# brown-palm/goal-force

Measured on AMD Instinct MI355X. Metric: frames_per_sec (81-frame video / (50-step denoise loop + VAE decode), Wan2.2-I2V-A14B 832x480x81f), higher is better.
Workload: dtype bf16

## Files before the change

### goal_force_amd/csrc/gf_abi.hip

```cpp
#include "gf_common.h"
#include <cstdarg>
#include <cstdio>
#include <cstdlib>
#include <cstring>

static thread_local char g_err[512] = "";

void gf_set_error(const char* fmt, ...) {
    va_list ap;
    va_start(ap, fmt);
    vsnprintf(g_err, sizeof(g_err), fmt, ap);
    va_end(ap);
}

extern "C" GF_API const char* gf_version(void) { return "goalforce-hip 0.1.0 gfx950"; }
extern "C" GF_API const char* gf_last_error(void) { return g_err; }
extern "C" GF_API int gf_abi_version(void) { return GF_ABI_VERSION; }

static GfOptions g_options;

const GfOptions& gf_options() { return g_options; }

namespace {
struct OptionSlot {
    const char* name;
    std::atomic<int> GfOptions::*field;
    int lo, hi, dflt;
};
const OptionSlot kSlots[] = {
    {"prefer_8wave", &GfOptions::prefer_8wave, 0, 1, 0}, {"a4_stagger", &GfOptions::a4_stagger, 0, 1 << 20, 2},
    {"a4_group_m", &GfOptions::a4_group_m, 0, 64, 0},    {"conv_nb", &GfOptions::conv_nb, 0, 2, 0},
    {"conv_gather", &GfOptions::conv_gather, 0, 1, 0},   {"vae_rms3", &GfOptions::vae_rms3, 0, 1, 1},
    {"conv_direct", &GfOptions::conv_direct, 0, 1, 1},
};
}

extern "C" GF_API int gf_set_option(const char* name, int value) {
    GF_CHECK_ARG(name, "gf_set_option: null name");
    for (const OptionSlot& s : kSlots)
        if (strcmp(name, s.name) == 0) {
            (g_options.*(s.field)).store(value < s.lo ? s.lo : (value > s.hi ? s.hi : value), std::memory_order_relaxed);
            return GF_OK;
        }
    gf_set_error("gf_set_option: unknown option '%s'", name);
    return GF_ERR_INVALID_ARG;
}

extern "C" GF_API int gf_get_option(const char* name, int* value) {
    GF_CHECK_ARG(name && value, "gf_get_option: null argument");
    for (const OptionSlot& s : kSlots)
        if (strcmp(name, s.name) == 0) {
            *value = (g_options.*(s.field)).load(std::memory_order_relaxed);
            return GF_OK;
        }
    gf_set_error("gf_get_option: unknown option '%s'", name);
    return GF_ERR_INVALID_ARG;
}

extern "C" GF_API void gf_reset_options(void) {
    for (const OptionSlot& s : kSlots) (g_options.*(s.field)).store(s.dflt, std::memory_order_relaxed);
}
```

### goal_force_amd/csrc/gf_attention.hip

```cpp
#include "gf_mfma_frame.h"
#include <cstdlib>

namespace {

constexpr int QB = 256;
constexpr int KVB = 64;
constexpr int HD = 128;
constexpr int KV_TILE_BYTES = KVB * HD * 2;

constexpr int K3_RING = 2;
constexpr int K3_DMA0 = 10;
constexpr int K3_DMAS = 8;

struct AttnArgs {
    const u16* q;
    const u16* k;
    const u16* v;
    u16* o;
    int q_len, kv_len, heads, n_qblocks;
    long q_stride, k_stride, v_stride, o_stride;
    float scale_log2e;
    unsigned long long* dbg;
    float* lse;
    const u16* vt;
    long kv_pad;
    float last_key_bias;
    const int* row_ptr;
    const int* tile_idx;
    const int* head_map;
    int n_maps;
};

constexpr int AT2_THREADS = 512;
constexpr int AT2_V_BASE = 2 * KV_TILE_BYTES;
constexpr int AT2_LDS = 4 * KV_TILE_BYTES;

__device__ __forceinline__ void mfma32(f32x16& acc, const bf16x8& a, const bf16x8& b) {
    acc = __builtin_amdgcn_mfma_f32_32x32x16_bf16(a, b, acc, 0, 0, 0);
}

template <bool VT>
__global__ __launch_bounds__(AT2_THREADS, 2) void flash_attn_fwd_kernel2(const AttnArgs p) {
    extern __shared__ __attribute__((aligned(16))) char smem[];
    GF_LDS char* lds = (GF_LDS char*)smem;
    const int tid = threadIdx.x;
    const int lane = tid & 63;
    const int wave = __builtin_amdgcn_readfirstlane(tid >> 6);
    const int r = lane & 31, h = lane >> 5;
    int head, qb;
    {
        const int pid = blockIdx.x;
        if ((p.heads & 7) == 0) {
            const int xcd = pid & 7, idx = pid >> 3;
            head = xcd + 8 * (idx / p.n_qblocks);
            qb = idx % p.n_qblocks;
        } else {
            head = pid / p.n_qblocks;
            qb = pid % p.n_qblocks;
        }
    }
    const int q0 = qb * QB + wave * 32;

    bf16x8 qf[8];
// ... 379 lines not shown
        GF_LDS char* ob = lds + wave * 8192;
#pragma unroll
        for (int d = 0; d < 4; ++d)
#pragma unroll
            for (int rg = 0; rg < 4; ++rg) {
                u32x2 pk;
                pk[0] = pack2bf(oacc[d][4 * rg + 0] * inv, oacc[d][4 * rg + 1] * inv);
                pk[1] = pack2bf(oacc[d][4 * rg + 2] * inv, oacc[d][4 * rg + 3] * inv);
                *(GF_LDS u32x2*)(ob + r * 256 + (((4 * d + rg) ^ (r & 15)) << 4) + 8 * h) = pk;
            }
        asm volatile("s_waitcnt lgkmcnt(0)" ::: "memory");
#pragma unroll
        for (int it = 0; it < 8; ++it) {
            const int row = 4 * it + (lane >> 4), ch = lane & 15;
            const u16x8 v8 = *(GF_LDS u16x8*)(ob + row * 256 + ((ch ^ (row & 15)) << 4));
            if (q0 + row < p.q_len)
                *reinterpret_cast<u16x8*>(p.o + (long)(q0 + row) * p.o_stride + head * HD + 8 * ch) = v8;
        }
    }
}

constexpr int K3_NQ = 2;
template <int NQ> struct At3 {
    static constexpr int WAVES = 16 / NQ, THREADS = 64 * WAVES, ROWS = 16 * NQ, PIECES = NQ;
    static constexpr int SLOTS = 32 * NQ;
};
constexpr int AT3_V_BASE = 2 * KV_TILE_BYTES;
constexpr int AT3_LDS = 4 * KV_TILE_BYTES;

__device__ __forceinline__ void mfma16(f32x4& acc, const bf16x8& a, const bf16x8& b) {
    acc = __builtin_amdgcn_mfma_f32_16x16x32_bf16(a, b, acc, 0, 0, 0);
}

template <int NQ, bool SPARSE>
__global__ __launch_bounds__(At3<NQ>::THREADS, (NQ == 2 ? 2 : 1)) void flash_attn_fwd_kernel3(const AttnArgs p) {
    constexpr int NP = At3<NQ>::PIECES, NW = At3<NQ>::WAVES, RW = At3<NQ>::ROWS, NS = At3<NQ>::SLOTS;
    extern __shared__ __attribute__((aligned(16))) char smem[];
    GF_LDS char* lds = (GF_LDS char*)smem;
    const int tid = threadIdx.x;
    const int lane = tid & 63;
    const int wave = __builtin_amdgcn_readfirstlane(tid >> 6);
    const int r = lane & 15, g = lane >> 4;
    int head, qb0;
    gf_xcd_head_block(blockIdx.x, p.heads, p.n_qblocks, head, qb0);
    const int q0 = qb0 * QB + wave * RW;

    int vt_last = 0;
    bf16x8 qf[NQ][4];
#pragma unroll
    for (int qb = 0; qb < NQ; ++qb) {
        const int qr = min(q0 + 16 * qb + r, p.q_len - 1);
        const u16* qp = p.q + (long)qr * p.q_stride + head * HD + 8 * g;
#pragma unroll
        for (int ks = 0; ks < 4; ++ks) {
            qf[qb][ks] = *reinterpret_cast<const bf16x8*>(qp + 32 * ks);
        }
    }

    const int dma_r = lane >> 4;
    unsigned k_off0, vt_off0;
    {
        const int row = 4 * wave + dma_r;
        const int lch = (lane & 15) ^ (row & 15);
        k_off0 = ((unsigned)row * (unsigned)p.k_stride + head * HD + lch * 8) * 2u;
        const int vrow = 8 * wave + (lane >> 3);
        const int vch = (lane & 7) ^ ((vrow >> 1) & 7);
        vt_off0 = (unsigned)(((long)head * HD + vrow) * p.kv_pad + vch * 8) * 2u;
    }
    const unsigned kstep = KVB * (unsigned)p.k_stride * 2u;
    const unsigned k_piece = 4u * NW * (unsigned)p.k_stride * 2u, vt_piece = 8u * NW * (unsigned)p.kv_pad * 2u;
    typedef __attribute__((ext_vector_type(4))) unsigned u32x4s;
    auto make_srd = [](const void* base) {
        const unsigned long b = (unsigned long)base;
        u32x4s s;
        s[0] = (unsigned)b;
        s[1] = (unsigned)(b >> 32) & 0xffffu;
        s[2] = 0xffffffffu;
        s[3] = 0x00020000u;
// ... 96 lines not shown
    };

    auto qk_plain = [&](auto par_c) __attribute__((always_inline)) {
        constexpr int PAR = decltype(par_c)::value;
#pragma unroll
        for (int kb = 0; kb < 4; ++kb)
#pragma unroll
            for (int qb = 0; qb < NQ; ++qb) sc[PAR][kb][qb] = negm[qb];
#pragma unroll
        for (int ks = 0; ks < 4; ++ks)
#pragma unroll
            for (int kb = 0; kb < 4; ++kb) {
                const bf16x8 kf = *(GF_LDS bf16x8*)(lds + koff[ks] + kb * 4096 + PAR * KV_TILE_BYTES);
#pragma unroll
                for (int qb = 0; qb < NQ; ++qb) mfma_qk(sc[PAR][kb][qb], kf, qf[qb][ks]);
            }
    };
    auto pv_plain = [&](auto buf_c) __attribute__((always_inline)) {
        constexpr int BUF = decltype(buf_c)::value;
#pragma unroll
        for (int kk = 0; kk < 2; ++kk)
#pragma unroll
            for (int db = 0; db < 8; ++db) {
                const bf16x8 vf = *(GF_LDS bf16x8*)(lds + voff[kk] + db * 2048 + BUF * KV_TILE_BYTES);
#pragma unroll
                for (int qb = 0; qb < NQ; ++qb) mfma_pv(oacc[db][qb], vf, pf(kk, qb));
            }
#pragma unroll
        for (int kk = 0; kk < 2; ++kk)
#pragma unroll
            for (int qb = 0; qb < NQ; ++qb) mfma_pv(oacc[NDB - 1][qb], ones, pf(kk, qb));
    };
    auto apply_pending = [&]() __attribute__((always_inline)) {
        if (pend) {
    #pragma unroll
            for (int db = 0; db < NDB; ++db)
#pragma unroll
                for (int qb = 0; qb < NQ; ++qb)
#pragma unroll
                    for (int e = 0; e < 4; ++e) oacc[db][qb][e] *= alpha_pend[qb];
            pend = false;
        }
    };
    auto new_max = [&](auto par_c, const float (&mx)[NQ], bool first) {
        constexpr int PAR = decltype(par_c)::value;
        float over = mx[0];
#pragma unroll
        for (int qb = 1; qb < NQ; ++qb) over = fmaxf(over, mx[qb]);
        constexpr float QUIET = 6.0f;
        const bool quiet = __all(over <= QUIET);
        if (first || !quiet) {
#pragma unroll
            for (int qb = 0; qb < NQ; ++qb) {
                float d = mx[qb];
                d = fmaxf(d, __shfl_xor(d, 16));
                d = fmaxf(d, __shfl_xor(d, 32));
                if (!first) d = fmaxf(d, 0.f);
                const float m_new = d - negm[qb][0];
                const float alpha = __builtin_amdgcn_exp2f(-d);
#pragma unroll
                for (int kb = 0; kb < 4; ++kb)
#pragma unroll
                    for (int e = 0; e < 4; ++e) sc[PAR][kb][qb][e] -= d;
#pragma unroll
                for (int e = 0; e < 4; ++e) negm[qb][e] = -m_new;
                alpha_pend[qb] = alpha;
            }
            pend = !first;
        }
    };
    auto mask_ragged = [&](auto par_c, int t) __attribute__((always_inline)) {
        constexpr int PAR = decltype(par_c)::value;
        if (ragged && t == (SPARSE ? nt_all : nt) - 1) {
#pragma unroll
            for (int kb = 0; kb < 4; ++kb)
#pragma unroll
                for (int j = 0; j < 4; ++j)
                    if (t * KVB + 16 * kb + 4 * g + j >= p.kv_len) {
#pragma unroll
                        for (int qb = 0; qb < NQ; ++qb) sc[PAR][kb][qb][j] = -INFINITY;
                    }
        }
    };
    auto softmax_plain = [&](auto par_c, int t, int pos) __attribute__((always_inline)) {
        constexpr int PAR = decltype(par_c)::value;
        mask_ragged(par_c, t);
        float mx[NQ];
#pragma unroll
        for (int qb = 0; qb < NQ; ++qb) {
            mx[qb] = sc[PAR][0][qb][0];
#pragma unroll
            for (int kb = 0; kb < 4; ++kb)
#pragma unroll
                for (int j = 0; j < 4; ++j) mx[qb] = fmaxf(mx[qb], sc[PAR][kb][qb][j]);
        }
        new_max(par_c, mx, pos == 0);
#pragma unroll
        for (int qb = 0; qb < NQ; ++qb) {
#pragma unroll
            for (int kb = 0; kb < 4; ++kb)
#pragma unroll
                for (int j = 0; j < 4; j += 2) {
                    const float p0 = __builtin_amdgcn_exp2f(sc[PAR][kb][qb][j]);
                    const float p1 = __builtin_amdgcn_exp2f(sc[PAR][kb][qb][j + 1]);
                    pfw[kb >> 1][qb][(kb & 1) * 2 + (j >> 1)] = pack2bf(p0, p1);
                }
        }
    };

    constexpr int RING = K3_RING;
    bf16x8 fr[RING];
    auto frag_load = [&](auto f_c, auto par_c) __attribute__((always_inline)) {
        constexpr int F = decltype(f_c)::value, PAR = decltype(par_c)::value;
        if constexpr (F < 16) {
            constexpr int kk = F >> 3, db = F & 7;
            fr[F % RING] = *(GF_LDS bf16x8*)(lds + voff[kk] + db * 2048 + (1 - PAR) * KV_TILE_BYTES);
        } else if constexpr (F < 32) {
            constexpr int ks = (F - 16) >> 2, kb = (F - 16) & 3;
            fr[F % RING] = *(GF_LDS bf16x8*)(lds + koff[ks] + kb * 4096 + (1 - PAR) * KV_TILE_BYTES);
        }
    };
    auto mfma_op = [&](auto s_c, auto par_c) __attribute__((always_inline)) {
        constexpr int S = decltype(s_c)::value, PAR = decltype(par_c)::value;
        constexpr int F = S / NQ, qb = (F & 1) ? NQ - 1 - S % NQ : S % NQ;
        if constexpr (F < 16) {
            constexpr int kk = F >> 3, db = F & 7;
            mfma_pv(oacc[db][qb], fr[F % RING], pf(kk, qb));
        } else {
            constexpr int ks = (F - 16) >> 2, kb = (F - 16) & 3;
            if constexpr (ks == 0) {
                mfma_qk_first(sc[1 - PAR][kb][qb], fr[F % RING], qf[qb][ks], negm[qb]);
            } else {
                mfma_qk(sc[1 - PAR][kb][qb], fr[F % RING], qf[qb][ks]);
            }
        }
    };
    auto dma_slot = [&](auto s_c, auto par_c, int tv, int tk) __attribute__((always_inline)) {
        constexpr int S = decltype(s_c)::value, PAR = decltype(par_c)::value;
        if constexpr (S >= K3_DMA0 && (S - K3_DMA0) % K3_DMAS == 0 && (S - K3_DMA0) / K3_DMAS < 2 * NP) {
            constexpr int i = (S - K3_DMA0) / K3_DMAS;
            if constexpr (i < NP) {
                stage_piece(1, tv, PAR, i);
            } else {
                stage_piece(0, tk, PAR, i - NP);
            }
        }
    };
    auto phase = [&](auto par_c, int pidx) __attribute__((always_inline)) {
        constexpr int PAR = decltype(par_c)::value;
        apply_pending();
        gf_static_for<0, RING - 1>([&](auto f_c) { frag_load(f_c, par_c); });
        float mx[NQ];
#pragma unroll
        for (int qb = 0; qb < NQ; ++qb) mx[qb] = -INFINITY;
        gf_static_for<0, 4 * NQ>([&](auto s_c) {
            constexpr int S = decltype(s_c)::value;
            mfma_op(s_c, par_c);
            if constexpr (S % NQ == 0) frag_load(std::integral_constant<int, S / NQ + RING - 1>{}, par_c);
            {
                constexpr int kb = S / NQ, qb = S % NQ;
                const f32x4& v = sc[PAR][kb][qb];
                mx[qb] = fmaxf(fmaxf(mx[qb], v[0]), v[1]);
                mx[qb] = fmaxf(fmaxf(mx[qb], v[2]), v[3]);
            }
            __builtin_amdgcn_sched_barrier(0);
        });
        new_max(par_c, mx, false);
        float pe[2];
        gf_static_for<4 * NQ, NS>([&](auto s_c) {
            constexpr int S = decltype(s_c)::value;
            mfma_op(s_c, par_c);
            if constexpr (S == 8 * NQ - 1 || S == 16 * NQ - 1) {
#pragma unroll
                for (int qb = 0; qb < NQ; ++qb) mfma_pv(oacc[NDB - 1][qb], ones, pf(S / (8 * NQ), qb));
            }
            if constexpr (S % NQ == 0) frag_load(std::integral_constant<int, S / NQ + RING - 1>{}, par_c);
            dma_slot(s_c, par_c, SPARSE ? w0 : pidx, SPARSE ? w2 : pidx + 2);
            if constexpr (S >= 8 * NQ) {
                constexpr int T = (S - 8 * NQ) % 3, e = ((S - 8 * NQ) / 3) * 2 + (T == 2 ? 1 : T);
                constexpr int kk = e / (8 * NQ), qb = (e >> 3) % NQ, kb = 2 * kk + ((e >> 2) & 1), j = e & 3;
                if constexpr (T != 2) {
                    asm volatile("v_exp_f32 %0, %1" : "=v"(pe[T]) : "v"(sc[PAR][kb][qb][j]));
                } else {
                    unsigned w;
                    asm volatile("v_cvt_pk_bf16_f32 %0, %1, %2" : "=v"(w) : "v"(pe[0]), "v"(pe[1]));
                    pfw[kk][qb][(kb & 1) * 2 + (j >> 1)] = w;
                }
            }
            __builtin_amdgcn_sched_barrier(0);
        });
        if constexpr (SPARSE) {
            w0 = w1;
            w1 = w2;
            w2 = tile_clamp(w_next);
            w_next = tile_raw(pidx + 4);
        }
        asm volatile("s_waitcnt vmcnt(0)" ::: "memory");
        __syncthreads();
    };

// ... 15 lines not shown
    if (nt > 1) qk_plain(C1{});
    asm volatile("s_waitcnt vmcnt(0)" ::: "memory");
    __syncthreads();
    int pi = 1;
    for (; pi + 1 <= nt - 2; pi += 2) {
        phase(C1{}, pi);
        phase(C0{}, pi + 1);
    }
    if (pi <= nt - 2) {
        phase(C1{}, pi);
        ++pi;
    }
    if (nt >= 2) {
        const int par = (nt - 1) & 1;
        const int t_last = SPARSE ? w0 : nt - 1;
        stage(1, t_last, par);
        apply_pending();
        if (par) {
            pv_plain(C0{});
            softmax_plain(C1{}, t_last, nt - 1);
        } else {
            pv_plain(C1{});
            softmax_plain(C0{}, t_last, nt - 1);
        }
        asm volatile("s_waitcnt vmcnt(0)" ::: "memory");
        __syncthreads();
    }
    apply_pending();
    if ((nt - 1) & 1)
        pv_plain(C1{});
    else
        pv_plain(C0{});

    {
        float inv[NQ];
#pragma unroll
        for (int qb = 0; qb < NQ; ++qb) {
            const float l = __shfl(oacc[NDB - 1][qb][0], r);
            inv[qb] = 1.0f / l;
            const int qrow = q0 + 16 * qb + r;
            if (p.lse && g == 0 && qrow < p.q_len) p.lse[(long)qrow * p.heads + head] = -negm[qb][0] + __builtin_amdgcn_logf(l);
        }
        __syncthreads();
        GF_LDS char* ob = lds + wave * (RW * 256);
#pragma unroll
        for (int qb = 0; qb < NQ; ++qb)
#pragma unroll
            for (int db = 0; db < 8; ++db) {
                u32x2 pk;
                pk[0] = pack2bf(oacc[db][qb][0] * inv[qb], oacc[db][qb][1] * inv[qb]);
                pk[1] = pack2bf(oacc[db][qb][2] * inv[qb], oacc[db][qb][3] * inv[qb]);
                const int row = 16 * qb + r;
                *(GF_LDS u32x2*)(ob + row * 256 + (((2 * db + (g >> 1)) ^ (row & 15)) << 4) + 8 * (g & 1)) = pk;
            }
        asm volatile("s_waitcnt lgkmcnt(0)" ::: "memory");
#pragma unroll
        for (int it = 0; it < RW / 4; ++it) {
            const int row = 4 * it + (lane >> 4), ch = lane & 15;
            const u16x8 v8 = *(GF_LDS u16x8*)(ob + row * 256 + ((ch ^ (row & 15)) << 4));
            if (q0 + row < p.q_len)
                *reinterpret_cast<u16x8*>(p.o + (long)(q0 + row) * p.o_stride + head * HD + 8 * ch) = v8;
        }
    }
}

__global__ __launch_bounds__(256) void transpose_v32_kernel(const u16* __restrict__ v, u16* __restrict__ vt, int kv_len, long kv_pad,
// ... 134 lines not shown
    GF_CHECK_ARG(v && vt, "gf_transpose_v: null pointer");
    GF_CHECK_ARG(kv_len > 0 && heads > 0 && kv_pad >= kv_len && kv_pad % KVB == 0 && v_stride % 8 == 0 && v_stride >= heads * HD,
                 "gf_transpose_v: kv_pad must be a multiple of 64 covering kv_len; v_stride must cover heads*128");
    GF_CHECK_ARG(gf_aligned16(v) && gf_aligned16(vt), "gf_transpose_v: 16-byte alignment required");
    GF_CHECK_ARG(heads * HD * kv_pad < (1LL << 31), "gf_transpose_v: heads*128*kv_pad must stay below 2^31 elements");
    hipLaunchKernelGGL(transpose_v_kernel, dim3((unsigned)(kv_pad / KVB), (unsigned)heads), dim3(256), 0, (hipStream_t)stream,
                       (const u16*)v, (u16*)vt, (int)kv_len, (long)kv_pad, (long)v_stride);
    GF_CHECK_LAUNCH("gf_transpose_v");
    return GF_OK;
}

extern "C" GF_API int gf_flash_attn_fwd_vt(const void* q, const void* k, const void* vt, void* o, float* lse, int64_t q_len,
                                           int64_t kv_len, int64_t kv_pad, int64_t heads, int64_t head_dim, int64_t q_stride,
                                           int64_t k_stride, int64_t o_stride, float scale, void* stream) {
    GF_CHECK_ARG(vt && kv_pad >= kv_len && kv_pad % KVB == 0 && gf_aligned16(vt), "gf_flash_attn_fwd_vt: bad V^T buffer");
    GF_CHECK_ARG(heads * HD * kv_pad < (1LL << 31), "gf_flash_attn_fwd_vt: heads*128*kv_pad must stay below 2^31 elements");
    return flash_attn_fwd_impl(q, k, k, o, lse, q_len, kv_len, heads, head_dim, q_stride, k_stride, k_stride, o_stride, scale,
                               stream, vt, kv_pad);
}

extern "C" GF_API int gf_transpose_v32(const void* v, int64_t v_stride, void* vt, int64_t kv_len, int64_t kv_pad, int64_t heads,
                                       void* stream) {
    GF_CHECK_ARG(v && vt, "gf_transpose_v32: null pointer");
    GF_CHECK_ARG(kv_len > 0 && heads > 0 && kv_pad >= kv_len && kv_pad % KVB == 0 && v_stride % 8 == 0 && v_stride >= heads * HD,
                 "gf_transpose_v32: kv_pad must be a multiple of 64 covering kv_len; v_stride must cover heads*128");
    GF_CHECK_ARG(gf_aligned16(v) && gf_aligned16(vt), "gf_transpose_v32: 16-byte alignment required");
    GF_CHECK_ARG(heads * HD * kv_pad < (1LL << 31), "gf_transpose_v32: heads*128*kv_pad must stay below 2^31 elements");
    hipLaunchKernelGGL(transpose_v32_kernel, dim3((unsigned)(kv_pad / KVB), (unsigned)heads), dim3(256), 0, (hipStream_t)stream,
                       (const u16*)v, (u16*)vt, (int)kv_len, (long)kv_pad, (long)v_stride);
    GF_CHECK_LAUNCH("gf_transpose_v32");
    return GF_OK;
}

static int flash_attn_vt32_impl(const char* fn, const void* q, const void* k, const void* vt, void* o, float* lse, const int32_t* row_ptr,
                                const int32_t* tile_idx, const int32_t* head_map, int64_t n_maps, int64_t q_len, int64_t kv_len,
                                int64_t kv_pad, int64_t heads, int64_t head_dim, int64_t q_stride, int64_t k_stride, int64_t o_stride,
                                float scale, void* stream) {
    GF_CHECK_ARG(q && k && vt && o, "%s: null pointer", fn);
    if (head_dim != HD) {
        gf_set_error("%s: head_dim=%ld unsupported (kernel is built for 128)", fn, (long)head_dim);
        return GF_ERR_UNSUPPORTED;
    }
    GF_CHECK_ARG(q_len >= 0 && kv_len >= 2 * KVB && heads > 0 && q_len < (1 << 30) && kv_len < (1 << 30),
                 "%s: bad lengths q=%ld kv=%ld heads=%ld (kv_len >= 128)", fn, (long)q_len, (long)kv_len, (long)heads);
    GF_CHECK_ARG(kv_pad >= kv_len && kv_pad % KVB == 0 && heads * HD * kv_pad < (1LL << 31), "%s: bad V^T buffer", fn);
    GF_CHECK_ARG(q_stride % 8 == 0 && k_stride % 8 == 0 && o_stride % 4 == 0 && q_stride >= heads * HD && k_stride >= heads * HD &&
                     o_stride >= heads * HD,
                 "%s: strides must cover heads*128 and be multiples of 8", fn);
    GF_CHECK_ARG(gf_aligned16(q) && gf_aligned16(k) && gf_aligned16(vt) && gf_aligned16(o), "%s: 16-byte alignment required", fn);
    GF_CHECK_ARG((kv_len + 64) * k_stride < (1LL << 31), "%s: kv_len*stride must stay below 2^31 elements", fn);
    const bool sparse = row_ptr != nullptr;
    const int64_t n_qblocks = (q_len + QB - 1) / QB;
    if (sparse)
        GF_CHECK_ARG(n_maps >= 1 && n_maps * n_qblocks < (1LL << 31) - 1, "%s: n_maps=%ld (at least 1; n_maps * query blocks below 2^31)", fn,
                     (long)n_maps);
    if (q_len == 0) return GF_OK;
    AttnArgs a;
    a.q = (const u16*)q;
    a.k = (const u16*)k;
    a.v = (const u16*)k;
    a.o = (u16*)o;
    a.q_len = (int)q_len;
    a.kv_len = (int)kv_len;
    a.heads = (int)heads;
    a.n_qblocks = (int)n_qblocks;
    a.q_stride = q_stride;
    a.k_stride = k_stride;
    a.v_stride = k_stride;
    a.o_stride = o_stride;
    a.scale_log2e = scale * 1.4426950408889634f;
    a.lse = lse;
    a.vt = (const u16*)vt;
    a.kv_pad = kv_pad;
    a.dbg = nullptr;
    a.last_key_bias = 0.f;
    a.row_ptr = row_ptr;
    a.tile_idx = tile_idx;
    a.head_map = head_map;
    a.n_maps = (int)n_maps;
    const dim3 grid((unsigned)(a.n_qblocks * a.heads)), block(At3<K3_NQ>::THREADS);
    return sparse ? gf_launch_lds<flash_attn_fwd_kernel3<K3_NQ, true>>(fn, GF_ATTR_MSG_PLAIN, fn, grid, block, AT3_LDS, (hipStream_t)stream, a)
                  : gf_launch_lds<flash_attn_fwd_kernel3<K3_NQ, false>>(fn, GF_ATTR_MSG_PLAIN, fn, grid, block, AT3_LDS, (hipStream_t)stream, a);
}

extern "C" GF_API int gf_flash_attn_fwd_vt32(const void* q, const void* k, const void* vt, void* o, float* lse, int64_t q_len,
                                             int64_t kv_len, int64_t kv_pad, int64_t heads, int64_t head_dim, int64_t q_stride,
                                             int64_t k_stride, int64_t o_stride, float scale, void* stream) {
    return flash_attn_vt32_impl("gf_flash_attn_fwd_vt32", q, k, vt, o, lse, nullptr, nullptr, nullptr, 0, q_len, kv_len, kv_pad, heads,
                                head_dim, q_stride, k_stride, o_stride, scale, stream);
}

extern "C" GF_API int gf_flash_attn_fwd_vt32_sparse(const void* q, const void* k, const void* vt, void* o, float* lse,
                                                    const int32_t* row_ptr, const int32_t* tile_idx, const int32_t* head_map,
                                                    int64_t n_maps, int64_t q_len, int64_t kv_len, int64_t kv_pad, int64_t heads,
                                                    int64_t head_dim, int64_t q_stride, int64_t k_stride, int64_t o_stride, float scale,
                                                    void* stream) {
    GF_CHECK_ARG(row_ptr && tile_idx, "gf_flash_attn_fwd_vt32_sparse: null map pointer");
    return flash_attn_vt32_impl("gf_flash_attn_fwd_vt32_sparse", q, k, vt, o, lse, row_ptr, tile_idx, head_map, n_maps, q_len, kv_len,
                                kv_pad, heads, head_dim, q_stride, k_stride, o_stride, scale, stream);
}
```

### goal_force_amd/csrc/gf_common.h

```cpp
#pragma once
#include <hip/hip_runtime.h>
#include <stdint.h>
#include "goalforce.h"

typedef unsigned short u16;
typedef __attribute__((ext_vector_type(8))) __bf16 bf16x8;
typedef __attribute__((ext_vector_type(4))) __bf16 bf16x4;
typedef __attribute__((ext_vector_type(8))) unsigned short u16x8;
typedef __attribute__((ext_vector_type(4))) unsigned short u16x4;
typedef __attribute__((ext_vector_type(4))) short s16x4;
typedef __attribute__((ext_vector_type(4))) float f32x4;
typedef __attribute__((ext_vector_type(16))) float f32x16;
typedef __attribute__((ext_vector_type(4))) unsigned int u32x4;
typedef __attribute__((ext_vector_type(2))) unsigned int u32x2;

#define GF_LDS __attribute__((address_space(3)))
#define GF_GLOBAL __attribute__((address_space(1)))

__device__ __forceinline__ float bf2f(u16 u) { return __uint_as_float(((unsigned)u) << 16); }
__device__ __forceinline__ u16 f2bf(float f) { return __builtin_bit_cast(u16, (__bf16)f); }
__device__ __forceinline__ float rbf(float f) { return bf2f(f2bf(f)); }
__device__ __forceinline__ unsigned pack2bf(float lo, float hi) {
    typedef __attribute__((ext_vector_type(2))) float f2_t;
    typedef __attribute__((ext_vector_type(2))) __bf16 b2_t;
// ... 36 lines not shown
    float t = 0.f;
#pragma unroll
    for (int i = 0; i < THREADS / 64; ++i) t += red[i];
    return t;
}

void gf_set_error(const char* fmt, ...);
#define GF_CHECK_ARG(cond, ...)                 \
    do {                                        \
        if (!(cond)) {                          \
            gf_set_error(__VA_ARGS__);          \
            return GF_ERR_INVALID_ARG;          \
        }                                       \
    } while (0)
#define GF_CHECK_LAUNCH(name)                                                        \
    do {                                                                             \
        hipError_t e_ = hipGetLastError();                                           \
        if (e_ != hipSuccess) {                                                      \
            gf_set_error("%s: launch failed: %s", name, hipGetErrorString(e_));      \
            return GF_ERR_LAUNCH;                                                    \
        }                                                                            \
    } while (0)
static inline bool gf_aligned16(const void* p) { return (((uintptr_t)p) & 15u) == 0; }

#include <atomic>
struct GfOptions {
    std::atomic<int> prefer_8wave{0};
    std::atomic<int> a4_stagger{2};
    std::atomic<int> a4_group_m{0};
    std::atomic<int> conv_nb{0};
    std::atomic<int> conv_gather{0};
    std::atomic<int> vae_rms3{1};
    std::atomic<int> conv_direct{1};
};
int gf_conv3d_direct_c96(const void* src_walk, const void* Wm, int64_t ldw, const void* bias, void* out, int64_t T_out, int64_t H,
                         int64_t W, int64_t N, int epilogue, const void* resid, const void* zero_page, void* stream);
int gf_conv2d_up_direct_c192(const void* src0, const void* Wm, int64_t ldw, const void* bias, void* out, int64_t T_out, int64_t Hs,
                             int64_t Ws, const void* zero_page, void* stream);
const GfOptions& gf_options();

#include <atomic>
#include <mutex>
struct GfDeviceOnce {
    std::atomic<uint64_t> done{0};
    std::mutex mu;
};
template <class F>
static inline hipError_t gf_once_per_device(GfDeviceOnce& st, F&& f) {
    int dev = 0;
    hipError_t e = hipGetDevice(&dev);
    if (e != hipSuccess) return e;
    if (dev < 0 || dev >= 64) return hipErrorInvalidDevice;
    const uint64_t bit = 1ull << dev;
    if (st.done.load(std::memory_order_acquire) & bit) return hipSuccess;
    std::lock_guard<std::mutex> lock(st.mu);
    if (st.done.load(std::memory_order_relaxed) & bit) return hipSuccess;
    e = f();
    if (e == hipSuccess) st.done.fetch_or(bit, std::memory_order_release);
    return e;
}
```

### goal_force_amd/ops.py

```python
from __future__ import annotations

import math

import torch

from . import _lib
from ._lib import (EPI_BIAS, EPI_BIAS_GATE_RESID, EPI_BIAS_GELU_TANH, EPI_BIAS_MUL, EPI_BIAS_RESID, EPI_BIAS_SILU,
                   GoalForceError)

__all__ = [
    "modulation", "layernorm_modulate", "rmsnorm_rope", "gate_residual", "gemm", "flash_attn", "flash_attn_sparse", "BlockMap", "patchify_im2col", "unpatchify",
    "cfg_euler_step", "act", "add", "sub", "rel_l1", "force_map",
    "EPI_BIAS", "EPI_BIAS_GELU_TANH", "EPI_BIAS_GATE_RESID", "EPI_BIAS_RESID", "EPI_BIAS_SILU", "EPI_BIAS_MUL",
]

_BF16 = torch.bfloat16
_FP8 = torch.float8_e4m3fn

PROFILE_ATTN = None
PROFILE_GEMM = None
PROFILE_CONV = None


def _stream(t: torch.Tensor):
# ... 187 lines not shown
    _lib.check(_lib.load().gf_rope_apply(_ptr(xv), _ptr(ov), _ptr(cos), _ptr(sin), rows, dim, head_dim, xs, os_, _stream(x)),
               "gf_rope_apply")
    return out


def _gemm(a, w, row_scale, bias, epilogue, resid, gate, out):
    av, M, K, lda, N, ldw = _linear_operands(a, w, row_scale)
    if out is None:
        out = torch.empty(a.shape[:-1] + (N,), dtype=_BF16, device=a.device)
    ov, Mo, No, ldc = _rows2d(out, "gemm[_fp8].out")
    if (Mo, No) != (M, N):
        raise GoalForceError(f"gemm[_fp8].out: expected [{M}, {N}], got [{Mo}, {No}]")
    ldr = 0
    if resid is not None:
        _req(resid, "gemm[_fp8].resid")
        resid, Mr, Nr, ldr = _rows2d(resid, "gemm[_fp8].resid")
        if (Mr, Nr) != (M, N):
            raise GoalForceError(f"gemm[_fp8].resid: expected [{M}, {N}], got [{Mr}, {Nr}]")
    _vec(gate, "gemm[_fp8].gate", N)
    _vec(bias, "gemm[_fp8].bias", N)
    lib = _lib.load()
    fn, scale = (lib.gf_gemm_bf16, ()) if row_scale is None else (lib.gf_gemm_fp8, (_ptr(row_scale),))
    with _timed(PROFILE_GEMM, M, N, K, int(epilogue)):
        _lib.check(fn(_ptr(av), lda, _ptr(w), ldw, *scale, _ptr(bias), _ptr(ov), ldc, M, N, K, int(epilogue), _ptr(resid), ldr,
                      _ptr(gate), _stream(a)), fn.__name__)
    return out


def gemm(a, w, bias=None, epilogue=EPI_BIAS, resid=None, gate=None, out=None):
    return _gemm(a, w, None, bias, epilogue, resid, gate, out)


VT_MIN_KV = 2048
_LIB_DEFAULTS = {"prefer_8wave": 0, "a4_stagger": 2, "a4_group_m": 0, "conv_nb": 0, "conv_gather": 0, "conv_direct": 1, "vae_rms3": 1}
_OPT = {"attn_k3": True, "vt_from_gemm": True, "conv_padded": True, "fold_pad_keys": True, "attn_q_prescale": True, "vae_attn_offset": True,
        "fold_cross_o": True}


def lib_option(name: str) -> int:
    import ctypes
    v = ctypes.c_int(0)
    _lib.check(_lib.load().gf_get_option(name.encode(), ctypes.byref(v)), f"gf_get_option({name})")
    return int(v.value)


class options:

    def __init__(self, **kv):
        for k in kv:
            if k not in _OPT and k not in _LIB_DEFAULTS:
                raise GoalForceError(f"ops.options: unknown option {k!r}")
        self.kv, self.old = kv, {}

    @staticmethod
    def _apply_one(k, v):
        if k in _OPT:
            _OPT[k] = bool(v)
        else:
            _lib.check(_lib.load().gf_set_option(k.encode(), int(v)), f"gf_set_option({k})")

    def __enter__(self):
        self.old = {}
        try:
            for k, v in self.kv.items():
                old = _OPT[k] if k in _OPT else lib_option(k)
                self._apply_one(k, v)
                self.old[k] = old
# ... 18 lines not shown
    if ws is None or ws.numel() < numel:
        ws = _VT_WS[key] = torch.empty((numel,), dtype=_BF16, device=device)
    return ws


def _vt_shape(skv, num_heads, head_dim):
    return skv >= VT_MIN_KV and head_dim == 128 and num_heads * 128 * kv_pad(skv) < 2 ** 31


def vt32_ok(skv, num_heads, head_dim):
    return _vt_shape(skv, num_heads, head_dim) and _OPT["attn_k3"] and _OPT["vt_from_gemm"]


def _linear_vt32(x, w, x_scale, bias):
    xv, skv, K, ldx, N, ldw = _linear_operands(x, w, x_scale)
    _vec(bias, "linear_vt32[_fp8].bias", N)
    vt = _vt_workspace(N * kv_pad(skv), x.device)
    lib = _lib.load()
    fn, scale = (lib.gf_linear_vt32, ()) if x_scale is None else (lib.gf_linear_vt32_fp8, (_ptr(x_scale),))
    _lib.check(fn(_ptr(xv), ldx, *scale, _ptr(w), ldw, _ptr(bias), _ptr(vt), skv, kv_pad(skv), N, K, _stream(x)), fn.__name__)
    return vt


def linear_vt32(x, weight, bias):
    return _linear_vt32(x, weight, None, bias)


def linear_vt32_fp8(x8, x_scale, w8, bias):
    if x_scale is None:
        raise GoalForceError("linear_vt32_fp8.x_scale: required")
    return _linear_vt32(x8, w8, x_scale, bias)


def _vt_attn(lib, q, k, v, vt, out, lse, sq, skv, num_heads, head_dim, scale, k3, block_map=None):
    tr, fa = (lib.gf_transpose_v32, lib.gf_flash_attn_fwd_vt32) if k3 else (lib.gf_transpose_v, lib.gf_flash_attn_fwd_vt)
    tiles = ()
    if block_map is not None:
        fa = lib.gf_flash_attn_fwd_vt32_sparse
        tiles = (_ptr(block_map.row_ptr), _ptr(block_map.tile_idx), _ptr(block_map.head_map), block_map.n_maps)
    if vt is None:
        vt = _vt_workspace(num_heads * 128 * kv_pad(skv), q.device)
        _lib.check(tr(_ptr(v), v.stride(0), _ptr(vt), skv, kv_pad(skv), num_heads, _stream(q)), "gf_transpose_v")
    _lib.check(fa(_ptr(q), _ptr(k), _ptr(vt), _ptr(out), _ptr(lse), *tiles, sq, skv, kv_pad(skv), num_heads, head_dim,
                  q.stride(0), k.stride(0), out.stride(0), float(scale), _stream(q)), fa.__name__ if tiles else "gf_flash_attn_fwd_vt")


def flash_attn(q, k, v, num_heads, out=None, scale=None, vt=None, last_key_mult=1, finished_q=False):
    for n, t in (("q", q), ("k", k)) + ((("v", v),) if vt is None else ()):
        _mat(t, f"flash_attn.{n}")
    sq, hd_all = q.shape
    skv = k.shape[0]
    head_dim = hd_all // num_heads
    if k.shape[1] != hd_all or (vt is None and v.shape != k.shape) or head_dim * num_heads != hd_all:
        raise GoalForceError("flash_attn: q/k/v shape mismatch")
    if vt is not None and not vt32_ok(skv, num_heads, head_dim):
        raise GoalForceError("flash_attn: a pre-transposed V is only taken by kernel 3 (key length >= VT_MIN_KV, head_dim 128)")
    if out is None:
        out = torch.empty((sq, hd_all), dtype=_BF16, device=q.device)
    if scale is None:
        scale = 1.0 / math.sqrt(head_dim)
    if last_key_mult != 1 and (vt is not None or skv >= VT_MIN_KV):
        raise GoalForceError("flash_attn: last_key_mult is for short key sequences (the text context), not the V^T path")
    long_keys = _vt_shape(skv, num_heads, head_dim)
    if finished_q and vt is not None:
        raise GoalForceError("flash_attn: finished_q goes to kernel 2, which does not take kernel 3's V^T operand")
    if vt is not None and vt.numel() < num_heads * 128 * kv_pad(skv):
        raise GoalForceError("flash_attn.vt: buffer smaller than heads*128*kv_pad")
    lib = _lib.load()
    with _timed(PROFILE_ATTN, sq, skv, num_heads):
        if long_keys:
            _vt_attn(lib, q, k, v, vt, out, None, sq, skv, num_heads, head_dim, scale, _OPT["attn_k3"] and not finished_q)
        elif last_key_mult != 1:
            _lib.check(lib.gf_flash_attn_fwd_lastmult(_ptr(q), _ptr(k), _ptr(v), _ptr(out), sq, skv, num_heads, head_dim, q.stride(0),
                                                      k.stride(0), v.stride(0), out.stride(0), float(scale), float(last_key_mult),
                                                      _stream(q)), "gf_flash_attn_fwd_lastmult")
        else:
            _lib.check(lib.gf_flash_attn_fwd(_ptr(q), _ptr(k), _ptr(v), _ptr(out), sq, skv, num_heads, head_dim,
# ... 769 lines not shown
```

### include/goalforce.h

```cpp
#ifndef GOALFORCE_H
#define GOALFORCE_H

#include <stdint.h>

#if defined(GF_BUILD)
#define GF_API __attribute__((visibility("default")))
#else
#define GF_API
#endif

#ifdef __cplusplus
extern "C" {
#endif

typedef enum {
    GF_OK = 0,
    GF_ERR_INVALID_ARG = -1,
    GF_ERR_UNSUPPORTED = -2,
    GF_ERR_LAUNCH = -3
} gf_status;

GF_API const char* gf_version(void);
GF_API const char* gf_last_error(void);
#define GF_ABI_VERSION 20
// ... 20 lines not shown
    GF_EPI_BIAS_GATE_RESID = 2,
    GF_EPI_BIAS_RESID = 3,
    GF_EPI_BIAS_SILU = 4,
    GF_EPI_BIAS_MUL = 5
} gf_epilogue;

GF_API int gf_gemm_bf16(const void* A, int64_t lda, const void* W, int64_t ldw, const void* bias,
                 void* C, int64_t ldc, int64_t M, int64_t N, int64_t K,
                 int epilogue, const void* resid, int64_t ldr, const void* gate,
                 void* stream);

GF_API int gf_gemm_bf16_batched(const void* A, int64_t lda, int64_t strideA, const void* W, int64_t ldw, int64_t strideW, void* C,
                                int64_t ldc, int64_t strideC, int64_t M, int64_t N, int64_t K, int64_t batch, void* stream);

GF_API int gf_flash_attn_fwd(const void* q, const void* k, const void* v, void* o,
                      int64_t q_len, int64_t kv_len, int64_t heads, int64_t head_dim,
                      int64_t q_stride, int64_t k_stride, int64_t v_stride, int64_t o_stride,
                      float scale, void* stream);

GF_API int gf_transpose_v(const void* v, int64_t v_stride, void* vt, int64_t kv_len, int64_t kv_pad, int64_t heads, void* stream);
GF_API int gf_flash_attn_fwd_vt(const void* q, const void* k, const void* vt, void* o, float* lse,
                         int64_t q_len, int64_t kv_len, int64_t kv_pad, int64_t heads, int64_t head_dim,
                         int64_t q_stride, int64_t k_stride, int64_t o_stride, float scale, void* stream);

GF_API int gf_transpose_v32(const void* v, int64_t v_stride, void* vt, int64_t kv_len, int64_t kv_pad, int64_t heads, void* stream);
GF_API int gf_flash_attn_fwd_vt32(const void* q, const void* k, const void* vt, void* o, float* lse,
                                  int64_t q_len, int64_t kv_len, int64_t kv_pad, int64_t heads, int64_t head_dim,
                                  int64_t q_stride, int64_t k_stride, int64_t o_stride, float scale, void* stream);

GF_API int gf_flash_attn_fwd_vt32_sparse(const void* q, const void* k, const void* vt, void* o, float* lse,
                                         const int32_t* row_ptr, const int32_t* tile_idx, const int32_t* head_map, int64_t n_maps,
                                         int64_t q_len, int64_t kv_len, int64_t kv_pad, int64_t heads, int64_t head_dim,
                                         int64_t q_stride, int64_t k_stride, int64_t o_stride, float scale, void* stream);

GF_API int gf_linear_vt32(const void* x, int64_t ldx, const void* w, int64_t ldw, const void* bias, void* vt,
                          int64_t kv_len, int64_t kv_pad, int64_t N, int64_t K, void* stream);

GF_API int gf_flash_attn_fwd_lastmult(const void* q, const void* k, const void* v, void* o, int64_t q_len, int64_t kv_len,
                                      int64_t heads, int64_t head_dim, int64_t q_stride, int64_t k_stride, int64_t v_stride,
                                      int64_t o_stride, float scale, float last_key_multiplicity, void* stream);

GF_API int gf_cross_probs(const void* q, const void* k, void* p, int64_t q_len, int64_t n_keys, int64_t n_pad, int64_t heads,
                          int64_t head_dim, int64_t q_stride, int64_t k_stride, int64_t p_stride, float scale,
                          float last_key_multiplicity, void* stream);

GF_API int gf_cross_fold_table(const void* v, const void* w_o, void* u, int64_t n_keys, int64_t n_pad, int64_t heads, int64_t head_dim,
                               int64_t n_out, int64_t v_stride, int64_t w_stride, int64_t u_stride, void* stream);

GF_API int gf_flash_attn_fwd_lse(const void* q, const void* k, const void* v, void* o, float* lse,
                          int64_t q_len, int64_t kv_len, int64_t heads, int64_t head_dim,
                          int64_t q_stride, int64_t k_stride, int64_t v_stride, int64_t o_stride,
                          float scale, void* stream);
GF_API int64_t gf_flash_attn_bwd_workspace_bytes(int64_t q_len, int64_t kv_len, int64_t heads);
GF_API int gf_flash_attn_bwd(const void* q, const void* k, const void* v, const void* o, const void* dout,
                      const float* lse, void* workspace, void* dq, void* dk, void* dv,
                      int64_t q_len, int64_t kv_len, int64_t heads, int64_t head_dim,
                      int64_t q_stride, int64_t k_stride, int64_t v_stride, int64_t o_stride, int64_t do_stride,
                      int64_t dq_stride, int64_t dk_stride, int64_t dv_stride, float scale, void* stream);

GF_API int gf_layernorm_bwd(const void* x, int64_t x_stride, const void* dy, int64_t dy_stride, const void* g, void* dx,
                            int64_t dx_stride, float* dg_acc, float* db_acc, int64_t rows, int64_t dim, float eps, void* stream);
GF_API int gf_rmsnorm_rope_bwd(const void* x, int64_t x_stride, const void* dy, int64_t dy_stride, const void* weight,
                               const float* cos_tab, const float* sin_tab, void* dx, int64_t dx_stride, float* dw_acc,
                               int64_t rows, int64_t dim, int64_t head_dim, float eps, void* stream);
GF_API int gf_colsum(const void* a, int64_t lda, const void* b, int64_t ldb, const void* gate, void* out, int64_t ldo,
                     float* acc, int64_t rows, int64_t cols, void* stream);
// ... 123 lines not shown
```

Before: 0.6302.

## Use fixed first-tile softmax max in attention with overflow-flagged repair pass

Adds a FIXED mode to the k3 flash-attention kernel, now the default. It takes the row max only from the first KV tile and then skips all later max reductions, new_max calls and output rescaling. After the PV loop it flags any wave whose accumulators hold inf or NaN. A second REPAIR launch exits early unless a wave in its block was flagged, and otherwise recomputes that block with the exact online softmax. The aim is to cut per-tile max/rescale ALU work in the long self-attention, at the cost of an extra launch, a flags workspace and possible precision loss when later scores far exceed the first-tile max without overflowing.

```diff
diff --git a/goal_force_amd/csrc/gf_abi.hip b/goal_force_amd/csrc/gf_abi.hip
--- a/goal_force_amd/csrc/gf_abi.hip
+++ b/goal_force_amd/csrc/gf_abi.hip
@@ -31,7 +31,7 @@
     {"prefer_8wave", &GfOptions::prefer_8wave, 0, 1, 0}, {"a4_stagger", &GfOptions::a4_stagger, 0, 1 << 20, 2},
     {"a4_group_m", &GfOptions::a4_group_m, 0, 64, 0},    {"conv_nb", &GfOptions::conv_nb, 0, 2, 0},
     {"conv_gather", &GfOptions::conv_gather, 0, 1, 0},   {"vae_rms3", &GfOptions::vae_rms3, 0, 1, 1},
-    {"conv_direct", &GfOptions::conv_direct, 0, 1, 1},
+    {"conv_direct", &GfOptions::conv_direct, 0, 1, 1},   {"attn_fixed_max", &GfOptions::attn_fixed_max, 0, 1, 1},
 };
 }
 
diff --git a/goal_force_amd/csrc/gf_attention.hip b/goal_force_amd/csrc/gf_attention.hip
--- a/goal_force_amd/csrc/gf_attention.hip
+++ b/goal_force_amd/csrc/gf_attention.hip
@@ -29,6 +29,7 @@
     const int* tile_idx;
     const int* head_map;
     int n_maps;
+    int* flags;
 };
 
 constexpr int AT2_THREADS = 512;
@@ -474,7 +475,8 @@
     acc = __builtin_amdgcn_mfma_f32_16x16x32_bf16(a, b, acc, 0, 0, 0);
 }
 
-template <int NQ, bool SPARSE>
+constexpr int K3_EXACT = 0, K3_FIXED = 1, K3_REPAIR = 2;
+template <int NQ, bool SPARSE, int MODE = K3_EXACT>
 __global__ __launch_bounds__(At3<NQ>::THREADS, (NQ == 2 ? 2 : 1)) void flash_attn_fwd_kernel3(const AttnArgs p) {
     constexpr int NP = At3<NQ>::PIECES, NW = At3<NQ>::WAVES, RW = At3<NQ>::ROWS, NS = At3<NQ>::SLOTS;
     extern __shared__ __attribute__((aligned(16))) char smem[];
@@ -486,6 +488,10 @@
     int head, qb0;
     gf_xcd_head_block(blockIdx.x, p.heads, p.n_qblocks, head, qb0);
     const int q0 = qb0 * QB + wave * RW;
+    if constexpr (MODE == K3_REPAIR) {
+        const int f = p.flags[((long)head * p.n_qblocks + qb0) * NW + (lane & (NW - 1))];
+        if (!__any(f != 0)) return;
+    }
 
     int vt_last = 0;
     bf16x8 qf[NQ][4];
@@ -648,6 +654,7 @@
             for (int qb = 0; qb < NQ; ++qb) mfma_pv(oacc[NDB - 1][qb], ones, pf(kk, qb));
     };
     auto apply_pending = [&]() __attribute__((always_inline)) {
+        if constexpr (MODE == K3_FIXED) return;
         if (pend) {
     #pragma unroll
             for (int db = 0; db < NDB; ++db)
@@ -701,16 +708,18 @@
     auto softmax_plain = [&](auto par_c, int t, int pos) __attribute__((always_inline)) {
         constexpr int PAR = decltype(par_c)::value;
         mask_ragged(par_c, t);
-        float mx[NQ];
-#pragma unroll
-        for (int qb = 0; qb < NQ; ++qb) {
-            mx[qb] = sc[PAR][0][qb][0];
-#pragma unroll
-            for (int kb = 0; kb < 4; ++kb)
-#pragma unroll
-                for (int j = 0; j < 4; ++j) mx[qb] = fmaxf(mx[qb], sc[PAR][kb][qb][j]);
-        }
-        new_max(par_c, mx, pos == 0);
+        if (MODE != K3_FIXED || pos == 0) {
+            float mx[NQ];
+#pragma unroll
+            for (int qb = 0; qb < NQ; ++qb) {
+                mx[qb] = sc[PAR][0][qb][0];
+#pragma unroll
+                for (int kb = 0; kb < 4; ++kb)
+#pragma unroll
+                    for (int j = 0; j < 4; ++j) mx[qb] = fmaxf(mx[qb], sc[PAR][kb][qb][j]);
+            }
+            new_max(par_c, mx, pos == 0);
+        }
 #pragma unroll
         for (int qb = 0; qb < NQ; ++qb) {
 #pragma unroll
@@ -773,7 +782,7 @@
             constexpr int S = decltype(s_c)::value;
             mfma_op(s_c, par_c);
             if constexpr (S % NQ == 0) frag_load(std::integral_constant<int, S / NQ + RING - 1>{}, par_c);
-            {
+            if constexpr (MODE != K3_FIXED) {
                 constexpr int kb = S / NQ, qb = S % NQ;
                 const f32x4& v = sc[PAR][kb][qb];
                 mx[qb] = fmaxf(fmaxf(mx[qb], v[0]), v[1]);
@@ -781,7 +790,7 @@
             }
             __builtin_amdgcn_sched_barrier(0);
         });
-        new_max(par_c, mx, false);
+        if constexpr (MODE != K3_FIXED) new_max(par_c, mx, false);
         float pe[2];
         gf_static_for<4 * NQ, NS>([&](auto s_c) {
             constexpr int S = decltype(s_c)::value;
@@ -863,6 +872,17 @@
     else
         pv_plain(C0{});
 
+    if constexpr (MODE == K3_FIXED) {
+        bool bad = false;
+#pragma unroll
+        for (int db = 0; db < NDB; ++db)
+#pragma unroll
+            for (int qb = 0; qb < NQ; ++qb)
+#pragma unroll
+                for (int e = 0; e < 4; ++e) bad |= __builtin_amdgcn_classf(oacc[db][qb][e], 0x207);
+        const int any_bad = __any(bad) ? 1 : 0;
+        if (lane == 0) p.flags[((long)head * p.n_qblocks + qb0) * NW + wave] = any_bad;
+    }
     {
         float inv[NQ];
 #pragma unroll
@@ -1063,7 +1083,12 @@
     return GF_OK;
 }
 
-static int flash_attn_vt32_impl(const char* fn, const void* q, const void* k, const void* vt, void* o, float* lse, const int32_t* row_ptr,
+template <bool SPARSE_K, int MODE>
+static int launch_k3(const char* fn, dim3 grid, dim3 block, hipStream_t stream, const AttnArgs& a) {
+    return gf_launch_lds<flash_attn_fwd_kernel3<K3_NQ, SPARSE_K, MODE>>(fn, GF_ATTR_MSG_PLAIN, fn, grid, block, AT3_LDS, stream, a);
+}
+
+static int flash_attn_vt32_impl(const char* fn, int32_t* flags, const void* q, const void* k, const void* vt, void* o, float* lse, const int32_t* row_ptr,
                                 const int32_t* tile_idx, const int32_t* head_map, int64_t n_maps, int64_t q_len, int64_t kv_len,
                                 int64_t kv_pad, int64_t heads, int64_t head_dim, int64_t q_stride, int64_t k_stride, int64_t o_stride,
                                 float scale, void* stream) {
@@ -1109,16 +1134,34 @@
     a.tile_idx = tile_idx;
     a.head_map = head_map;
     a.n_maps = (int)n_maps;
+    a.flags = flags;
     const dim3 grid((unsigned)(a.n_qblocks * a.heads)), block(At3<K3_NQ>::THREADS);
-    return sparse ? gf_launch_lds<flash_attn_fwd_kernel3<K3_NQ, true>>(fn, GF_ATTR_MSG_PLAIN, fn, grid, block, AT3_LDS, (hipStream_t)stream, a)
-                  : gf_launch_lds<flash_attn_fwd_kernel3<K3_NQ, false>>(fn, GF_ATTR_MSG_PLAIN, fn, grid, block, AT3_LDS, (hipStream_t)stream, a);
+    hipStream_t st = (hipStream_t)stream;
+    if (!flags) return sparse ? launch_k3<true, K3_EXACT>(fn, grid, block, st, a) : launch_k3<false, K3_EXACT>(fn, grid, block, st, a);
+    if (!gf_options().attn_fixed_max.load(std::memory_order_relaxed)) {
+        if (hipMemsetAsync(flags, 0, sizeof(int32_t) * (size_t)(n_qblocks * heads * At3<K3_NQ>::WAVES), st) != hipSuccess) {
+            gf_set_error("%s: hipMemsetAsync(flags) failed", fn);
+            return GF_ERR_LAUNCH;
+        }
+        return sparse ? launch_k3<true, K3_EXACT>(fn, grid, block, st, a) : launch_k3<false, K3_EXACT>(fn, grid, block, st, a);
+    }
+    if (const int rc = sparse ? launch_k3<true, K3_FIXED>(fn, grid, block, st, a) : launch_k3<false, K3_FIXED>(fn, grid, block, st, a)) return rc;
+    return sparse ? launch_k3<true, K3_REPAIR>(fn, grid, block, st, a) : launch_k3<false, K3_REPAIR>(fn, grid, block, st, a);
 }
 
 extern "C" GF_API int gf_flash_attn_fwd_vt32(const void* q, const void* k, const void* vt, void* o, float* lse, int64_t q_len,
                                              int64_t kv_len, int64_t kv_pad, int64_t heads, int64_t head_dim, int64_t q_stride,
                                              int64_t k_stride, int64_t o_stride, float scale, void* stream) {
-    return flash_attn_vt32_impl("gf_flash_attn_fwd_vt32", q, k, vt, o, lse, nullptr, nullptr, nullptr, 0, q_len, kv_len, kv_pad, heads,
+    return flash_attn_vt32_impl("gf_flash_attn_fwd_vt32", nullptr, q, k, vt, o, lse, nullptr, nullptr, nullptr, 0, q_len, kv_len, kv_pad, heads,
                                 head_dim, q_stride, k_stride, o_stride, scale, stream);
+}
+
+extern "C" GF_API int gf_flash_attn_fwd_vt32_fm(const void* q, const void* k, const void* vt, void* o, float* lse, int32_t* flags,
+                                                int64_t q_len, int64_t kv_len, int64_t kv_pad, int64_t heads, int64_t head_dim,
+                                                int64_t q_stride, int64_t k_stride, int64_t o_stride, float scale, void* stream) {
+    GF_CHECK_ARG(flags && ((uintptr_t)flags & 3u) == 0, "gf_flash_attn_fwd_vt32_fm: null or misaligned flags workspace");
+    return flash_attn_vt32_impl("gf_flash_attn_fwd_vt32_fm", flags, q, k, vt, o, lse, nullptr, nullptr, nullptr, 0, q_len, kv_len, kv_pad,
+                                heads, head_dim, q_stride, k_stride, o_stride, scale, stream);
 }
 
 extern "C" GF_API int gf_flash_attn_fwd_vt32_sparse(const void* q, const void* k, const void* vt, void* o, float* lse,
@@ -1127,6 +1170,17 @@
                                                     int64_t head_dim, int64_t q_stride, int64_t k_stride, int64_t o_stride, float scale,
                                                     void* stream) {
     GF_CHECK_ARG(row_ptr && tile_idx, "gf_flash_attn_fwd_vt32_sparse: null map pointer");
-    return flash_attn_vt32_impl("gf_flash_attn_fwd_vt32_sparse", q, k, vt, o, lse, row_ptr, tile_idx, head_map, n_maps, q_len, kv_len,
+    return flash_attn_vt32_impl("gf_flash_attn_fwd_vt32_sparse", nullptr, q, k, vt, o, lse, row_ptr, tile_idx, head_map, n_maps, q_len, kv_len,
                                 kv_pad, heads, head_dim, q_stride, k_stride, o_stride, scale, stream);
 }
+
+extern "C" GF_API int gf_flash_attn_fwd_vt32_sparse_fm(const void* q, const void* k, const void* vt, void* o, float* lse, int32_t* flags,
+                                                       const int32_t* row_ptr, const int32_t* tile_idx, const int32_t* head_map,
+                                                       int64_t n_maps, int64_t q_len, int64_t kv_len, int64_t kv_pad, int64_t heads,
+                                                       int64_t head_dim, int64_t q_stride, int64_t k_stride, int64_t o_stride,
+                                                       float scale, void* stream) {
+    GF_CHECK_ARG(row_ptr && tile_idx, "gf_flash_attn_fwd_vt32_sparse_fm: null map pointer");
+    GF_CHECK_ARG(flags && ((uintptr_t)flags & 3u) == 0, "gf_flash_attn_fwd_vt32_sparse_fm: null or misaligned flags workspace");
+    return flash_attn_vt32_impl("gf_flash_attn_fwd_vt32_sparse_fm", flags, q, k, vt, o, lse, row_ptr, tile_idx, head_map, n_maps, q_len,
+                                kv_len, kv_pad, heads, head_dim, q_stride, k_stride, o_stride, scale, stream);
+}
diff --git a/goal_force_amd/csrc/gf_common.h b/goal_force_amd/csrc/gf_common.h
--- a/goal_force_amd/csrc/gf_common.h
+++ b/goal_force_amd/csrc/gf_common.h
@@ -92,6 +92,7 @@
     std::atomic<int> conv_gather{0};
     std::atomic<int> vae_rms3{1};
     std::atomic<int> conv_direct{1};
+    std::atomic<int> attn_fixed_max{1};
 };
 int gf_conv3d_direct_c96(const void* src_walk, const void* Wm, int64_t ldw, const void* bias, void* out, int64_t T_out, int64_t H,
                          int64_t W, int64_t N, int epilogue, const void* resid, const void* zero_page, void* stream);
diff --git a/goal_force_amd/ops.py b/goal_force_amd/ops.py
--- a/goal_force_amd/ops.py
+++ b/goal_force_amd/ops.py
@@ -243,7 +243,8 @@
 
 
 VT_MIN_KV = 2048
-_LIB_DEFAULTS = {"prefer_8wave": 0, "a4_stagger": 2, "a4_group_m": 0, "conv_nb": 0, "conv_gather": 0, "conv_direct": 1, "vae_rms3": 1}
+_LIB_DEFAULTS = {"prefer_8wave": 0, "a4_stagger": 2, "a4_group_m": 0, "conv_nb": 0, "conv_gather": 0, "conv_direct": 1, "vae_rms3": 1,
+                 "attn_fixed_max": 1}
 _OPT = {"attn_k3": True, "vt_from_gemm": True, "conv_padded": True, "fold_pad_keys": True, "attn_q_prescale": True, "vae_attn_offset": True,
         "fold_cross_o": True}
 
@@ -328,17 +329,28 @@
     return _linear_vt32(x8, w8, x_scale, bias)
 
 
+last_attn_flags = None
+
+
 def _vt_attn(lib, q, k, v, vt, out, lse, sq, skv, num_heads, head_dim, scale, k3, block_map=None):
+    global last_attn_flags
     tr, fa = (lib.gf_transpose_v32, lib.gf_flash_attn_fwd_vt32) if k3 else (lib.gf_transpose_v, lib.gf_flash_attn_fwd_vt)
-    tiles = ()
+    tiles, flags = (), ()
+    last_attn_flags = None
+    fixed = k3 and lib_option("attn_fixed_max") != 0
+    if fixed:
+        fa = lib.gf_flash_attn_fwd_vt32_fm
+        last_attn_flags = torch.empty((num_heads, -(-sq // 256), 8), dtype=torch.int32, device=q.device)
+        flags = (_ptr(last_attn_flags),)
     if block_map is not None:
-        fa = lib.gf_flash_attn_fwd_vt32_sparse
+        fa = lib.gf_flash_attn_fwd_vt32_sparse_fm if fixed else lib.gf_flash_attn_fwd_vt32_sparse
         tiles = (_ptr(block_map.row_ptr), _ptr(block_map.tile_idx), _ptr(block_map.head_map), block_map.n_maps)
     if vt is None:
         vt = _vt_workspace(num_heads * 128 * kv_pad(skv), q.device)
         _lib.check(tr(_ptr(v), v.stride(0), _ptr(vt), skv, kv_pad(skv), num_heads, _stream(q)), "gf_transpose_v")
-    _lib.check(fa(_ptr(q), _ptr(k), _ptr(vt), _ptr(out), _ptr(lse), *tiles, sq, skv, kv_pad(skv), num_heads, head_dim,
-                  q.stride(0), k.stride(0), out.stride(0), float(scale), _stream(q)), fa.__name__ if tiles else "gf_flash_attn_fwd_vt")
+    _lib.check(fa(_ptr(q), _ptr(k), _ptr(vt), _ptr(out), _ptr(lse), *flags, *tiles, sq, skv, kv_pad(skv), num_heads, head_dim,
+                  q.stride(0), k.stride(0), out.stride(0), float(scale), _stream(q)),
+               fa.__name__ if tiles or flags else "gf_flash_attn_fwd_vt")
 
 
 def flash_attn(q, k, v, num_heads, out=None, scale=None, vt=None, last_key_mult=1, finished_q=False):
diff --git a/include/goalforce.h b/include/goalforce.h
--- a/include/goalforce.h
+++ b/include/goalforce.h
@@ -76,6 +76,14 @@
                                          const int32_t* row_ptr, const int32_t* tile_idx, const int32_t* head_map, int64_t n_maps,
                                          int64_t q_len, int64_t kv_len, int64_t kv_pad, int64_t heads, int64_t head_dim,
                                          int64_t q_stride, int64_t k_stride, int64_t o_stride, float scale, void* stream);
+
+GF_API int gf_flash_attn_fwd_vt32_fm(const void* q, const void* k, const void* vt, void* o, float* lse, int32_t* flags,
+                                     int64_t q_len, int64_t kv_len, int64_t kv_pad, int64_t heads, int64_t head_dim,
+                                     int64_t q_stride, int64_t k_stride, int64_t o_stride, float scale, void* stream);
+GF_API int gf_flash_attn_fwd_vt32_sparse_fm(const void* q, const void* k, const void* vt, void* o, float* lse, int32_t* flags,
+                                            const int32_t* row_ptr, const int32_t* tile_idx, const int32_t* head_map, int64_t n_maps,
+                                            int64_t q_len, int64_t kv_len, int64_t kv_pad, int64_t heads, int64_t head_dim,
+                                            int64_t q_stride, int64_t k_stride, int64_t o_stride, float scale, void* stream);
 
 GF_API int gf_linear_vt32(const void* x, int64_t ldx, const void* w, int64_t ldw, const void* bias, void* vt,
                           int64_t kv_len, int64_t kv_pad, int64_t N, int64_t K, void* stream);
```

Measured after the change: 0.6435, median of 6. 2.1% higher.
